# hongsukchoi/Pose2Mesh_RELEASE

Measured on NVIDIA H100. Metric: SMPL meshes/sec, higher is better.
Workload: dtype f32 (wgmma fp16x3 split, fp32 accumulate)

## Files before the change

pose2mesh_release_b200/csrc/cheb_umma.cu:

```cuda
#include <cuda.h>
#include <cuda_fp16.h>
#include <cuda_runtime.h>

#include <algorithm>
#include <cstdlib>
#include <cstring>
#include <vector>

#include "p2m_internal.h"

namespace p2m {

namespace {

constexpr int TILE_M = 128;
constexpr int FC = 32;
constexpr int A_BLOCK_BYTES = TILE_M * 128;
constexpr float W_SCALE = 64.f;
constexpr float W_INV_SCALE = 1.f / 64.f;

struct TileHeader {
  int n_rows;
  int h1;
  int nnz;
  int off_halo;
  int off_rp;
  int off_ent;
  int off_ord2;
  int bytes;
  int pad[8];
};
static_assert(sizeof(TileHeader) == 64, "header size");

inline int up16(int x) { return (x + 15) & ~15; }

__device__ __forceinline__ uint32_t smem_u32(const void* p) { return (uint32_t)__cvta_generic_to_shared(p); }

__device__ __forceinline__ void mbar_init(uint32_t bar, uint32_t count) {
  asm volatile("mbarrier.init.shared::cta.b64 [%0], %1;" ::"r"(bar), "r"(count));
}
__device__ __forceinline__ void mbar_arrive(uint32_t bar) {
  asm volatile("mbarrier.arrive.shared::cta.b64 _, [%0];" ::"r"(bar) : "memory");
}
__device__ __forceinline__ void mbar_arrive_expect_tx(uint32_t bar, uint32_t bytes) {
  asm volatile("mbarrier.arrive.expect_tx.shared::cta.b64 _, [%0], %1;" ::"r"(bar), "r"(bytes) : "memory");
}
__device__ __forceinline__ bool mbar_try_wait(uint32_t bar, uint32_t parity) {
  uint32_t ok;
  asm volatile(
      "{\n\t.reg .pred p;\n\t"
      "mbarrier.try_wait.parity.shared::cta.b64 p, [%1], %2, %3;\n\t"
      "selp.u32 %0, 1, 0, p;\n\t}"
      : "=r"(ok)
      : "r"(bar), "r"(parity), "r"(20000u)
      : "memory");
  return ok != 0;
}
__device__ __forceinline__ unsigned long long global_ns() {
  unsigned long long t;
  asm volatile("mov.u64 %0, %globaltimer;" : "=l"(t));
  return t;
}
constexpr unsigned long long MBAR_TIMEOUT_NS = 2000000000ull;
__device__ __noinline__ void mbar_timeout(volatile int* abort_flag, int* status, int code) {
  *abort_flag = 1;
  *reinterpret_cast<volatile int*>(status) = code;
  __threadfence_system();
}
__device__ __forceinline__ void mbar_wait(uint32_t bar, uint32_t parity, volatile int* abort_flag, int* status,
                                          int code) {
  if (mbar_try_wait(bar, parity)) return;
  unsigned long long t0 = 0;
  for (unsigned spin = 0;; ++spin) {
#pragma unroll 1
    for (int it = 0; it < 64; ++it) {
      if (mbar_try_wait(bar, parity)) return;
    }
    if (*abort_flag) return;
    if ((spin & 63u) == 63u) {
      const unsigned long long t = global_ns();
      if (t0 == 0) t0 = t;
      else if (t - t0 > MBAR_TIMEOUT_NS) break;
    }
  }
  mbar_timeout(abort_flag, status, code);
}
template <unsigned SLEEP_NS = 200>
__device__ __forceinline__ void mbar_wait_relaxed(uint32_t bar, uint32_t parity, volatile int* abort_flag, int* status,
                                                  int code) {
  if (mbar_try_wait(bar, parity)) return;
  unsigned long long t0 = 0;
  for (unsigned spin = 0;; ++spin) {
#pragma unroll 1
    for (int it = 0; it < 16; ++it) {
      if (mbar_try_wait(bar, parity)) return;
      __nanosleep(SLEEP_NS);
    }
    if (*abort_flag) return;
    if ((spin & 255u) == 255u) {
      const unsigned long long t = global_ns();
      if (t0 == 0) t0 = t;
      else if (t - t0 > MBAR_TIMEOUT_NS) break;
    }
  }
  mbar_timeout(abort_flag, status, code);
}
__device__ __forceinline__ void fence_barrier_init() { asm volatile("fence.mbarrier_init.release.cluster;" ::: "memory"); }
__device__ __forceinline__ void fence_async_proxy() { asm volatile("fence.proxy.async.shared::cta;" ::: "memory"); }

__device__ __forceinline__ void bulk_g2s(uint32_t dst, const void* src, uint32_t bytes, uint32_t bar) {
  asm volatile("cp.async.bulk.shared::cluster.global.mbarrier::complete_tx::bytes [%0], [%1], %2, [%3];" ::"r"(dst),
               "l"(src), "r"(bytes), "r"(bar)
               : "memory");
}
__device__ __forceinline__ void cp_async16(uint32_t dst, const void* src) {
  asm volatile("cp.async.cg.shared.global [%0], [%1], 16;" ::"r"(dst), "l"(src) : "memory");
}
__device__ __forceinline__ void cp_async16_zfill(uint32_t dst, const void* src, uint32_t src_bytes) {
  asm volatile("cp.async.cg.shared.global [%0], [%1], 16, %2;" ::"r"(dst), "l"(src), "r"(src_bytes) : "memory");
}
__device__ __forceinline__ void tma_load_2d(uint32_t dst, const CUtensorMap* tm, int c0, int c1, uint32_t bar) {
  asm volatile(
      "cp.async.bulk.tensor.2d.shared::cluster.global.mbarrier::complete_tx::bytes [%0], [%1, {%2, %3}], [%4];" ::"r"(dst),
      "l"(reinterpret_cast<uint64_t>(tm)), "r"(c0), "r"(c1), "r"(bar)
      : "memory");
}
__device__ __forceinline__ void prefetch_l2(const void* ptr) {
  asm volatile("prefetch.global.L2 [%0];" ::"l"(ptr));
}
__device__ __forceinline__ void cp_async_arrive_noinc(uint32_t bar) {
  asm volatile("cp.async.mbarrier.arrive.noinc.shared::cta.b64 [%0];" ::"r"(bar) : "memory");
}
__device__ __forceinline__ void producer_barrier() { asm volatile("bar.sync 1, 512;" ::: "memory"); }
__device__ __forceinline__ float4 lds_f4(uint32_t a) {
  float4 v;
  asm volatile("ld.shared.v4.f32 {%0, %1, %2, %3}, [%4];" : "=f"(v.x), "=f"(v.y), "=f"(v.z), "=f"(v.w) : "r"(a));
  return v;
}
__device__ __forceinline__ uint2 lds_u2(uint32_t a) {
  uint2 v;
  asm volatile("ld.shared.v2.u32 {%0, %1}, [%2];" : "=r"(v.x), "=r"(v.y) : "r"(a));
  return v;
}
__device__ __forceinline__ uint32_t lds_u16(uint32_t a) {
  unsigned short v;
  asm volatile("ld.shared.u16 %0, [%1];" : "=h"(v) : "r"(a));
  return v;
}
__device__ __forceinline__ void sts_f4(uint32_t a, const float4& v) {
  asm volatile("st.shared.v4.f32 [%0], {%1, %2, %3, %4};" ::"r"(a), "f"(v.x), "f"(v.y), "f"(v.z), "f"(v.w) : "memory");
}
__device__ __forceinline__ void sts_f2(uint32_t a, float x, float y) {
  asm volatile("st.shared.v2.f32 [%0], {%1, %2};" ::"r"(a), "f"(x), "f"(y) : "memory");
}
__device__ __forceinline__ void sts_u2(uint32_t a, const uint2& v) {
  asm volatile("st.shared.v2.u32 [%0], {%1, %2};" ::"r"(a), "r"(v.x), "r"(v.y) : "memory");
}
__device__ __forceinline__ void fma4(float4& acc, float w, const float4& x) {
  acc.x = fmaf(w, x.x, acc.x);
  acc.y = fmaf(w, x.y, acc.y);
  acc.z = fmaf(w, x.z, acc.z);
  acc.w = fmaf(w, x.w, acc.w);
}
__device__ __forceinline__ float4 cheb_t2(const float4& g, const float4& x) {
  return make_float4(fmaf(2.f, g.x, -x.x), fmaf(2.f, g.y, -x.y), fmaf(2.f, g.z, -x.z), fmaf(2.f, g.w, -x.w));
}
__device__ __forceinline__ float4 gather_row4(uint32_t ent, uint32_t e, uint32_t e1, uint32_t rows_q) {
  float4 acc0 = make_float4(0.f, 0.f, 0.f, 0.f), acc1 = acc0;
  for (; e + 3 < e1; e += 4) {
    const uint2 a0 = lds_u2(ent + e * 8), a1 = lds_u2(ent + e * 8 + 8), a2 = lds_u2(ent + e * 8 + 16),
                a3 = lds_u2(ent + e * 8 + 24);
    const float4 x0 = lds_f4(rows_q + a0.x), x1 = lds_f4(rows_q + a1.x), x2 = lds_f4(rows_q + a2.x),
                 x3 = lds_f4(rows_q + a3.x);
    fma4(acc0, __uint_as_float(a0.y), x0);
    fma4(acc1, __uint_as_float(a1.y), x1);
    fma4(acc0, __uint_as_float(a2.y), x2);
    fma4(acc1, __uint_as_float(a3.y), x3);
  }
  if (e + 1 < e1) {
    const uint2 a0 = lds_u2(ent + e * 8), a1 = lds_u2(ent + e * 8 + 8);
    const float4 x0 = lds_f4(rows_q + a0.x), x1 = lds_f4(rows_q + a1.x);
    fma4(acc0, __uint_as_float(a0.y), x0);
    fma4(acc1, __uint_as_float(a1.y), x1);
    e += 2;
  }
  if (e < e1) {
    const uint2 a0 = lds_u2(ent + e * 8);
    fma4(acc0, __uint_as_float(a0.y), lds_f4(rows_q + a0.x));
  }
  return make_float4(acc0.x + acc1.x, acc0.y + acc1.y, acc0.z + acc1.z, acc0.w + acc1.w);
}

__device__ __forceinline__ void wg_fence() { asm volatile("wgmma.fence.sync.aligned;" ::: "memory"); }
__device__ __forceinline__ void wg_commit() { asm volatile("wgmma.commit_group.sync.aligned;" ::: "memory"); }
__device__ __forceinline__ void wg_wait0() { asm volatile("wgmma.wait_group.sync.aligned 0;" ::: "memory"); }
template <int TA, int TB>
__device__ __forceinline__ void wgmma_m64n64(float (&d)[32], uint64_t desc_a, uint64_t desc_b) {
  asm volatile(
      "{\n\t.reg .pred p;\n\tsetp.ne.b32 p, 1, 0;\n\t"
      "wgmma.mma_async.sync.aligned.m64n64k16.f32.f16.f16 "
      "{%0, %1, %2, %3, %4, %5, %6, %7, %8, %9, %10, %11, %12, %13, %14, %15, "
      "%16, %17, %18, %19, %20, %21, %22, %23, %24, %25, %26, %27, %28, %29, %30, %31}, %32, %33, p, 1, 1, %34, %35;\n\t}"
      : "+f"(d[0]), "+f"(d[1]), "+f"(d[2]), "+f"(d[3]), "+f"(d[4]), "+f"(d[5]), "+f"(d[6]), "+f"(d[7]), "+f"(d[8]),
        "+f"(d[9]), "+f"(d[10]), "+f"(d[11]), "+f"(d[12]), "+f"(d[13]), "+f"(d[14]), "+f"(d[15]), "+f"(d[16]),
        "+f"(d[17]), "+f"(d[18]), "+f"(d[19]), "+f"(d[20]), "+f"(d[21]), "+f"(d[22]), "+f"(d[23]), "+f"(d[24]),
        "+f"(d[25]), "+f"(d[26]), "+f"(d[27]), "+f"(d[28]), "+f"(d[29]), "+f"(d[30]), "+f"(d[31])
      : "l"(desc_a), "l"(desc_b), "n"(TA), "n"(TB)
      : "memory");
}
template <int TA, int TB>
__device__ __forceinline__ void wgmma_m64n32(float (&d)[16], uint64_t desc_a, uint64_t desc_b) {
  asm volatile(
      "{\n\t.reg .pred p;\n\tsetp.ne.b32 p, 1, 0;\n\t"
      "wgmma.mma_async.sync.aligned.m64n32k16.f32.f16.f16 "
      "{%0, %1, %2, %3, %4, %5, %6, %7, %8, %9, %10, %11, %12, %13, %14, %15}, %16, %17, p, 1, 1, %18, %19;\n\t}"
      : "+f"(d[0]), "+f"(d[1]), "+f"(d[2]), "+f"(d[3]), "+f"(d[4]), "+f"(d[5]), "+f"(d[6]), "+f"(d[7]), "+f"(d[8]),
        "+f"(d[9]), "+f"(d[10]), "+f"(d[11]), "+f"(d[12]), "+f"(d[13]), "+f"(d[14]), "+f"(d[15])
      : "l"(desc_a), "l"(desc_b), "n"(TA), "n"(TB)
      : "memory");
// ... 28 lines not shown
struct KParams {
  const float* x;
  int in_unpool;
  int V, P, fin;
  int n_tiles;
  const unsigned char* meta;
  const int* meta_bytes;
  int meta_stride, max_h1;
  const unsigned char* wpack;
  const float* zero_row;
  EpiDev ep;
  int res_identity;
  const float* t1;
  const float* a_scale;
  long long ldy;
  int y_col0;
  float* y;
  int* status;
  long long* trace;
  int own_table;
  const float* head_wt;
  float* head_z;
  const unsigned char* apack;
  long long wslice_bytes;
  long long wblock_stride;
  int tma;
  CUtensorMap tm_x, tm_t1;
};

#ifdef P2M_UMMA_TRACE
__device__ __forceinline__ void trace_ev(const KParams& p, int role, int& n, int ev) {
  if (p.trace != nullptr && blockIdx.x == 0 && blockIdx.y == 0 && n < 512) {
    p.trace[role * 512 + n] = ((long long)ev << 48) | (clock64() & 0xFFFFFFFFFFFFll);
    ++n;
  }
}
#else
__device__ __forceinline__ void trace_ev(const KParams&, int, int&, int) {}
#endif

constexpr int W_PROD = 16;
constexpr int W_XLOAD = 16, N_XLOAD = 2, W_BLOAD = 18, W_EPI0 = 20;
constexpr int NUM_THREADS2 = 24 * 32;
constexpr int REGS_LAUNCH = 80, REGS_UTIL = 40, REGS_EPI = 120;
static_assert(128 * (REGS_EPI - REGS_LAUNCH) <= 128 * (REGS_LAUNCH - REGS_UTIL), "register pool balance");
static_assert(W_XLOAD % 4 == 0 && W_EPI0 % 4 == 0 && W_EPI0 - W_XLOAD == 4, "setmaxnreg works on aligned warpgroups");

template <int N>
__host__ __device__ constexpr int tile_rows() { return N == 128 ? 64 : TILE_M; }
template <int N, int NS, int XS, int MODE>
__global__ void __launch_bounds__(NUM_THREADS2, 1) k_cheb_conv_umma(const __grid_constant__ KParams p) {
  static_assert(N == 64 || N == 128, "one warpgroup holds the CTA's 128 x 64 or 64 x 128 accumulator in registers");
  constexpr int TM = tile_rows<N>();
  constexpr int RPT = TM / 64;
  constexpr int H = TM / 64;
  constexpr int ER = 16 * H;
  constexpr bool KT1 = (MODE == 1);
  constexpr bool plain = !KT1;
  constexpr bool XDIRECT = KT1 && NS >= 3;
  constexpr int A_BYTES = TM * 128;
  constexpr int B_BLOCK_BYTES = N * 128;
  constexpr int SLOT_BYTES = A_BYTES + B_BLOCK_BYTES;

  extern __shared__ __align__(1024) unsigned char smem_raw[];
  unsigned char* ring = smem_raw;
  float* Xs = reinterpret_cast<float*>(ring + NS * SLOT_BYTES);
  const size_t xs_stage_floats = (XDIRECT && TM == 64) ? 0 : (size_t)TM * FC;
  float* T1s = Xs + XS * xs_stage_floats;
  const size_t t1_stage_floats = (size_t)p.max_h1 * FC;
  unsigned char* meta_s =
      reinterpret_cast<unsigned char*>(T1s + (plain ? 0 : XS) * t1_stage_floats);
  uint64_t* bars = reinterpret_cast<uint64_t*>(meta_s + 2 * (size_t)p.meta_stride);
  uint64_t* b_ab_full = bars;
  uint64_t* b_ab_empty = b_ab_full + NS;
  uint64_t* b_x_full = b_ab_empty + NS;
  uint64_t* b_x_empty = b_x_full + XS;
  uint64_t* b_m_full = b_x_empty + XS;
  uint64_t* b_m_empty = b_m_full + 2;
  uint32_t* flags = reinterpret_cast<uint32_t*>(b_m_empty + 2);
  volatile int* abort_flag = reinterpret_cast<volatile int*>(flags + 1);
  float* ep_mul = reinterpret_cast<float*>(flags + 4);
  float* ep_add = ep_mul + N;
  constexpr int EC = 32;
  constexpr int STG_WARP_BYTES = N == 128 ? 4 * 16 * EC * 4 : 32 * EC * 4;
  unsigned char* epi_stage =
      reinterpret_cast<unsigned char*>((reinterpret_cast<uintptr_t>(ep_add + N) + 127) & ~(uintptr_t)127);
  int* own_s = reinterpret_cast<int*>(epi_stage + 4 * STG_WARP_BYTES);
  float* head_w_s = reinterpret_cast<float*>(own_s + 4 * 32);

  const int tid = threadIdx.x;
  const int warp = tid >> 5;
  const int lane = tid & 31;
  const int n_chunk = p.fin / FC;
  const int n_use = 3 * n_chunk;

  if (tid == 0) {
    for (int s = 0; s < NS; ++s) {
      mbar_init(smem_u32(b_ab_full + s), p.apack != nullptr ? 1 : W_PROD + 1);
      mbar_init(smem_u32(b_ab_empty + s), 4);
    }
    for (int s = 0; s < XS; ++s) {
      mbar_init(smem_u32(b_x_full + s), N_XLOAD * 32 + 1);
      mbar_init(smem_u32(b_x_empty + s), 1);
    }
    for (int s = 0; s < 2; ++s) {
      mbar_init(smem_u32(b_m_full + s), 1);
      mbar_init(smem_u32(b_m_empty + s), 1);
    }
    *abort_flag = (smem_u32(ring) & 1023u) ? 1 : 0;
    if (*abort_flag) mbar_timeout(abort_flag, p.status, 100);
    fence_barrier_init();
  }
  const float a_scale = p.a_scale ? *p.a_scale : 1.f;
  const int ecol0 = (int)blockIdx.y * N;
  for (int n = threadIdx.x; n < N; n += NUM_THREADS2) {
    const float sc = (p.ep.scale ? p.ep.scale[ecol0 + n] : 1.f) / a_scale;
    const float sh = p.ep.scale ? p.ep.shift[ecol0 + n] : 0.f;
    const float bi = p.ep.bias ? p.ep.bias[ecol0 + n] : 0.f;
    ep_mul[n] = W_INV_SCALE * sc;
    ep_add[n] = fmaf(bi, p.ep.scale ? p.ep.scale[ecol0 + n] : 1.f, sh);
  }
  if (N == 64 && p.head_z != nullptr)
    for (int i = threadIdx.x; i < 64 * 12; i += NUM_THREADS2) head_w_s[i] = p.head_wt[i];
  __syncthreads();

  if (warp >= W_XLOAD && warp < W_EPI0) {
  asm volatile("setmaxnreg.dec.sync.aligned.u32 %0;" ::"n"(REGS_UTIL));
  if (warp >= W_XLOAD && warp < W_XLOAD + N_XLOAD) {
    if (p.apack == nullptr) {
      const int lt = tid - W_XLOAD * 32;
      const int lq = lt & 7, lrg = lt >> 3;
      const int my_tiles = (p.n_tiles - (int)blockIdx.x + (int)gridDim.x - 1) / (int)gridDim.x;
      if (lt == 32 && p.tma) {
        if (!XDIRECT) asm volatile("prefetch.tensormap [%0];" ::"l"(reinterpret_cast<uint64_t>(&p.tm_x)) : "memory");
        if (KT1) asm volatile("prefetch.tensormap [%0];" ::"l"(reinterpret_cast<uint64_t>(&p.tm_t1)) : "memory");
      }
      auto fetch_meta = [&](int itf) {
        const int pat = (blockIdx.x + itf * gridDim.x) % p.P;
        const int m = itf & 1;
        mbar_wait_relaxed(smem_u32(b_m_empty + m), ((itf >> 1) & 1) ^ 1, abort_flag, p.status, 1);
        const int mbytes = p.meta_bytes[pat];
        mbar_arrive_expect_tx(smem_u32(b_m_full + m), mbytes);
        bulk_g2s(smem_u32(meta_s + (size_t)m * p.meta_stride), p.meta + (size_t)pat * p.meta_stride, mbytes,
                 smem_u32(b_m_full + m));
      };
      if (lt == 0 && my_tiles > 0) fetch_meta(0);
      const uint32_t fin_bytes = (uint32_t)p.fin * 4u;
      const int sh = p.in_unpool ? 1 : 0;
      int g2 = 0;
      int ltn = 0;
      for (int it2 = 0; it2 < my_tiles; ++it2) {
        const int tile2 = blockIdx.x + it2 * gridDim.x;
        const long long mesh_row0 = (long long)(tile2 / p.P) * p.V;
        const int m2 = it2 & 1;
        mbar_wait_relaxed(smem_u32(b_m_full + m2), (it2 >> 1) & 1, abort_flag, p.status, 8);
        const unsigned char* mb2 = meta_s + (size_t)m2 * p.meta_stride;
        const TileHeader* hdr2 = reinterpret_cast<const TileHeader*>(mb2);
        const int* halo = reinterpret_cast<const int*>(mb2 + hdr2->off_halo);
        const int h1 = hdr2->h1;
        for (int c2 = 0; c2 < n_chunk; ++c2, ++g2) {
          const int xs2 = g2 % XS;
          mbar_wait_relaxed(smem_u32(b_x_empty + xs2), ((g2 / XS) & 1) ^ 1, abort_flag, p.status, 11);
          if (lt == 0) trace_ev(p, 4, ltn, 1);
          const uint32_t xbar = smem_u32(b_x_full + xs2);
          auto stage_rows = [&](uint32_t dbase, const char* sbase, int first, int n_rows, int shift) {
            for (int i0 = first + lrg; i0 < n_rows; i0 += 32) {
              int v[4];
#pragma unroll
              for (int u = 0; u < 4; ++u) v[u] = (i0 + 8 * u < n_rows) ? halo[i0 + 8 * u] : -2;
#pragma unroll
              for (int u = 0; u < 4; ++u) {
                if (v[u] != -2) {
                  const uint32_t srow = (uint32_t)max(v[u], 0) >> shift;
                  cp_async16_zfill(dbase + (i0 + 8 * u) * 128, sbase + (uint64_t)srow * (uint64_t)fin_bytes,
                                   v[u] >= 0 ? 16u : 0u);
                }
              }
            }
          };
          const char* t1_mesh =
              reinterpret_cast<const char*>(KT1 ? p.t1 + mesh_row0 * p.fin + c2 * FC + lq * 4 : nullptr);
          const char* x_mesh = reinterpret_cast<const char*>(p.x + (mesh_row0 >> sh) * p.fin + c2 * FC + lq * 4);
          const uint32_t t1_dst = smem_u32(T1s + xs2 * t1_stage_floats) + lq * 16;
          const uint32_t x_dst = smem_u32(Xs + xs2 * xs_stage_floats) + lq * 16;
          if (p.tma) {
            if (lt == 32) {
              const int own0 = tile2 * TM;
              mbar_arrive_expect_tx(xbar, (XDIRECT ? 0 : (p.in_unpool ? TM / 2 : TM) * 128) + (KT1 ? TM * 128 : 0));
              if (!XDIRECT)
                tma_load_2d(smem_u32(Xs + xs2 * xs_stage_floats), &p.tm_x, c2 * FC, p.in_unpool ? own0 >> 1 : own0, xbar);
              if (KT1) tma_load_2d(smem_u32(T1s + xs2 * t1_stage_floats), &p.tm_t1, c2 * FC, own0, xbar);
            }
            if (KT1) stage_rows(t1_dst, t1_mesh, TM, h1, 0);
          } else {
            if (KT1) stage_rows(t1_dst, t1_mesh, 0, h1, 0);
            if (!XDIRECT) stage_rows(x_dst, x_mesh, 0, TM, sh);
            if (lt == 32) mbar_arrive(xbar);
          }
          cp_async_arrive_noinc(xbar);
          if (lt == 0) trace_ev(p, 4, ltn, 2);
          if (lt == 0 && c2 == (n_chunk > 1 ? 1 : 0) && it2 + 1 < my_tiles) fetch_meta(it2 + 1);
        }
      }
    }
  } else if (warp == W_BLOAD) {
    if (lane == 0) {
      uint32_t ucnt = 0;
      int tn = 0;
      const int uses = plain ? n_chunk : n_use;
      for (int tile = blockIdx.x; tile < p.n_tiles; tile += gridDim.x) {
        for (int u = 0; u < uses; ++u, ++ucnt) {
          const int s = ucnt % NS;
          const uint32_t par = (ucnt / NS) & 1;
          mbar_wait_relaxed(smem_u32(b_ab_empty + s), par ^ 1, abort_flag, p.status, 4);
          trace_ev(p, 1, tn, 10 + u);
          const unsigned char* wsl = p.wpack + (size_t)blockIdx.y * (size_t)p.wslice_bytes;
          if (p.apack != nullptr) {
            mbar_arrive_expect_tx(smem_u32(b_ab_full + s), B_BLOCK_BYTES + A_BYTES);
            bulk_g2s(smem_u32(ring + s * SLOT_BYTES), p.apack + ((size_t)tile * uses + u) * A_BYTES, A_BYTES,
                     smem_u32(b_ab_full + s));
          } else {
            mbar_arrive_expect_tx(smem_u32(b_ab_full + s), B_BLOCK_BYTES);
          }
          bulk_g2s(smem_u32(ring + s * SLOT_BYTES + A_BYTES), wsl + (size_t)u * (size_t)p.wblock_stride, B_BLOCK_BYTES,
                   smem_u32(b_ab_full + s));
        }
      }
    }
  }
  } else if (warp >= W_EPI0) {
    asm volatile("setmaxnreg.inc.sync.aligned.u32 %0;" ::"n"(REGS_EPI));
    const int wq = warp - W_EPI0;
    constexpr int CPR = EC / 4;
    constexpr int RPI = 32 / CPR;
    const uint32_t stg = smem_u32(epi_stage) + (uint32_t)wq * STG_WARP_BYTES;
    const int prow = lane / CPR, pc = lane % CPR;
    constexpr int NP = ER / RPI;
    int colk[2];
#pragma unroll
    for (int k = 0; k < 2; ++k) colk[k] = (int)(((uint32_t)pc ^ (uint32_t)((k * RPI + prow) & 7)) << 2);
    const int trow = (lane >> 4) * 64 + wq * 16 + (lane & 15);
    const int uses = plain ? n_chunk : n_use;
    uint32_t ucnt = 0;
    int it = 0;
    int etn = 0;
    for (int tile = blockIdx.x; tile < p.n_tiles; tile += gridDim.x, ++it) {
      const int b = tile / p.P, pat = tile - b * p.P;
      const long long mesh0 = (long long)b * p.V;
      int* own_w = own_s + wq * 32;
      {
        int v;
        if (lane >= ER) {
          v = -1;
        } else if (p.own_table) {
          v = __ldg(reinterpret_cast<const int*>(p.meta + (size_t)pat * p.meta_stride + 64) + trow);
        } else {
          v = pat * TM + trow;
          if (v >= p.V) v = -1;
        }
        __syncwarp();
        own_w[lane] = v;
        __syncwarp();
      }
      int own_v[NP];
#pragma unroll
      for (int i = 0; i < NP; ++i) own_v[i] = own_w[i * RPI + prow];
      if (p.ep.res != nullptr) {
        const int lpr = ((p.apack != nullptr ? N : p.ep.res_F) * 4 + 127) >> 7;
        for (int j = lane; j < ER * lpr; j += 32) {
          const int rr = j / lpr, ln = j - rr * lpr;
          const int vtx = own_w[rr];
          if (vtx >= 0) {
            const long long r = mesh0 + vtx;
            prefetch_l2(p.ep.res + (p.ep.res_unpool ? (r >> 1) : r) * p.ep.res_F + (p.apack != nullptr ? ecol0 : 0) + ln * 32);
          }
        }
      }
      float acc[2][32];
#pragma unroll
      for (int h = 0; h < 2; ++h)
#pragma unroll
        for (int j = 0; j < 32; ++j) acc[h][j] = 0.f;
      if (wq == 0 && lane == 0) trace_ev(p, 3, etn, 1);
      for (int u = 0; u < uses; ++u, ++ucnt) {
        const uint32_t s = ucnt % NS;
        if (wq == 0 && lane == 0) trace_ev(p, 3, etn, 4);
        mbar_wait(smem_u32(b_ab_full + s), (ucnt / NS) & 1, abort_flag, p.status, 6);
        if (wq == 0 && lane == 0) trace_ev(p, 3, etn, 5);
        const uint32_t a0 = smem_u32(ring + s * SLOT_BYTES);
        wg_fence();
#pragma unroll
        for (int h = 0; h < 2; ++h) {
          const uint64_t da = make_desc_sw128(a0 + (TM == 128 ? (uint32_t)h * (64 * 128) : 0u));
          const uint64_t db = make_desc_sw128(a0 + A_BYTES + (TM == 64 ? (uint32_t)h * (64 * 128) : 0u));
          wgmma_m64n64<0, 0>(acc[h], da + 0, db + 0);
          wgmma_m64n64<0, 0>(acc[h], da + 2, db + 2);
          wgmma_m64n64<0, 0>(acc[h], da + 4, db + 0);
          wgmma_m64n64<0, 0>(acc[h], da + 6, db + 2);
          wgmma_m64n64<0, 0>(acc[h], da + 0, db + 4);
          wgmma_m64n64<0, 0>(acc[h], da + 2, db + 6);
        }
        wg_commit();
        wg_wait0();
        __syncwarp();
        if (lane == 0) mbar_arrive(smem_u32(b_ab_empty + s));
      }
      if (wq == 0 && lane == 0) trace_ev(p, 3, etn, 2);
      auto stage_slab = [&](int cb) {
        const uint32_t sb = stg + (N == 128 ? (uint32_t)(cb / 32) * (16 * EC * 4) : 0u);
#pragma unroll
        for (int h = 0; h < H; ++h)
#pragma unroll
          for (int jj = 0; jj < 4; ++jj)
#pragma unroll
            for (int r = 0; r < 2; ++r) {
              const int lr = 16 * h + (lane >> 2) + 8 * r;
              const int cc = 8 * jj + 2 * (lane & 3);
              const int ah = TM == 128 ? h : cb / 64;
              const int j = 4 * ((TM == 128 ? cb : cb % 64) / 8 + jj) + 2 * r;
              sts_f2(sb + lr * (EC * 4) + ((((uint32_t)(cc >> 2)) ^ (uint32_t)(lr & 7)) << 4) + (cc & 3) * 4,
                     acc[ah][j], acc[ah][j + 1]);
            }
        __syncwarp();
      };
      if (N == 64 && p.head_z != nullptr) {
        float z[12];
#pragma unroll
        for (int j = 0; j < 12; ++j) z[j] = 0.f;
#pragma unroll
        for (int cb = 0; cb < N; cb += 32) {
          stage_slab(cb);
#pragma unroll
          for (int c = 0; c < 8; ++c) {
            const float4 a = lds_f4(stg + lane * (EC * 4) + (((uint32_t)c ^ (uint32_t)(lane & 7)) << 4));
            const float av[4] = {a.x, a.y, a.z, a.w};
#pragma unroll
            for (int e = 0; e < 4; ++e) {
              const int n = cb + 4 * c + e;
              float t = fmaf(av[e], ep_mul[n], ep_add[n]);
              if (p.ep.relu) t = fmaxf(t, 0.f);
              const float4 w0 = *reinterpret_cast<const float4*>(head_w_s + n * 12);
              const float4 w1 = *reinterpret_cast<const float4*>(head_w_s + n * 12 + 4);
              const float4 w2 = *reinterpret_cast<const float4*>(head_w_s + n * 12 + 8);
              z[0] = fmaf(t, w0.x, z[0]); z[1] = fmaf(t, w0.y, z[1]); z[2] = fmaf(t, w0.z, z[2]); z[3] = fmaf(t, w0.w, z[3]);
              z[4] = fmaf(t, w1.x, z[4]); z[5] = fmaf(t, w1.y, z[5]); z[6] = fmaf(t, w1.z, z[6]); z[7] = fmaf(t, w1.w, z[7]);
              z[8] = fmaf(t, w2.x, z[8]); z[9] = fmaf(t, w2.y, z[9]); z[10] = fmaf(t, w2.z, z[10]); z[11] = fmaf(t, w2.w, z[11]);
            }
          }
          __syncwarp();
        }
        if (own_w[lane] >= 0) {
          float4* zr = reinterpret_cast<float4*>(p.head_z + (mesh0 + own_w[lane]) * 12);
          zr[0] = make_float4(z[0], z[1], z[2], z[3]);
          zr[1] = make_float4(z[4], z[5], z[6], z[7]);
          zr[2] = make_float4(z[8], z[9], z[10], z[11]);
        }
      } else if (N == 128) {
#pragma unroll
        for (int cb = 0; cb < N; cb += 32) stage_slab(cb);
        const bool res_id = p.ep.res != nullptr && p.res_identity;
        float4 rv[N / 32][NP];
#pragma unroll
        for (int cb = 0; cb < N; cb += 32)
#pragma unroll
          for (int i = 0; i < NP; ++i) {
            rv[cb / 32][i] = make_float4(0.f, 0.f, 0.f, 0.f);
            if (res_id && own_v[i] >= 0) {
              const long long r = mesh0 + own_v[i];
              rv[cb / 32][i] = __ldg(reinterpret_cast<const float4*>(
                  p.ep.res + (p.ep.res_unpool ? (r >> 1) : r) * p.ep.res_F + ecol0 + cb + colk[i & 1]));
            }
          }
#pragma unroll
        for (int cb = 0; cb < N; cb += 32) {
          const uint32_t sb = stg + (uint32_t)(cb / 32) * (16 * EC * 4);
          float4 mu_k[2], ad_k[2];
#pragma unroll
          for (int k = 0; k < 2; ++k) {
            mu_k[k] = *reinterpret_cast<const float4*>(ep_mul + cb + colk[k]);
            ad_k[k] = *reinterpret_cast<const float4*>(ep_add + cb + colk[k]);
          }
#pragma unroll
          for (int i = 0; i < NP; ++i) {
            const int rr = i * RPI + prow;
            const int gn = ecol0 + cb + colk[i & 1];
            const float4 a = lds_f4(sb + rr * (EC * 4) + (pc << 4));
            const int vtx = own_v[i];
            if (vtx >= 0) {
              const float4 mu = mu_k[i & 1], ad = ad_k[i & 1];
              float o[4] = {fmaf(a.x, mu.x, ad.x), fmaf(a.y, mu.y, ad.y), fmaf(a.z, mu.z, ad.z), fmaf(a.w, mu.w, ad.w)};
              if (p.ep.relu) {
#pragma unroll
                for (int e = 0; e < 4; ++e) o[e] = fmaxf(o[e], 0.f);
              }
              const long long r = mesh0 + vtx;
              if (p.ep.res != nullptr) {
                if (p.res_identity) {
                  o[0] += rv[cb / 32][i].x; o[1] += rv[cb / 32][i].y; o[2] += rv[cb / 32][i].z; o[3] += rv[cb / 32][i].w;
                } else {
                  const float* res_row = p.ep.res + (p.ep.res_unpool ? (r >> 1) : r) * p.ep.res_F;
#pragma unroll
                  for (int e = 0; e < 4; ++e) {
                    const float l = __ldg(p.ep.lam + gn + e);
                    o[e] += (1.f - l) * __ldg(res_row + __ldg(p.ep.i0 + gn + e)) + l * __ldg(res_row + __ldg(p.ep.i1 + gn + e));
                  }
                }
              }
              *reinterpret_cast<float4*>(p.y + r * p.ldy + p.y_col0 + gn) = make_float4(o[0], o[1], o[2], o[3]);
            }
          }
        }
        __syncwarp();
      } else {
#pragma unroll
        for (int cb = 0; cb < N; cb += 32) {
          stage_slab(cb);
          float4 mu_k[2], ad_k[2];
#pragma unroll
          for (int k = 0; k < 2; ++k) {
            mu_k[k] = *reinterpret_cast<const float4*>(ep_mul + cb + colk[k]);
            ad_k[k] = *reinterpret_cast<const float4*>(ep_add + cb + colk[k]);
          }
#pragma unroll
          for (int i = 0; i < NP; ++i) {
            const int rr = i * RPI + prow;
            const int n = cb + colk[i & 1];
            const int gn = ecol0 + n;
            const float4 a = lds_f4(stg + rr * (EC * 4) + (pc << 4));
            const int vtx = own_v[i];
            if (vtx >= 0) {
              const float4 mu = mu_k[i & 1], ad = ad_k[i & 1];
              float o[4] = {fmaf(a.x, mu.x, ad.x), fmaf(a.y, mu.y, ad.y), fmaf(a.z, mu.z, ad.z), fmaf(a.w, mu.w, ad.w)};
              if (p.ep.relu) {
#pragma unroll
                for (int e = 0; e < 4; ++e) o[e] = fmaxf(o[e], 0.f);
              }
              const long long r = mesh0 + vtx;
              if (p.ep.res != nullptr) {
                const float* res_row = p.ep.res + (p.ep.res_unpool ? (r >> 1) : r) * p.ep.res_F;
                if (p.res_identity) {
                  const float4 rv = __ldg(reinterpret_cast<const float4*>(res_row + gn));
                  o[0] += rv.x; o[1] += rv.y; o[2] += rv.z; o[3] += rv.w;
                } else {
#pragma unroll
                  for (int e = 0; e < 4; ++e) {
                    const float l = __ldg(p.ep.lam + gn + e);
                    o[e] += (1.f - l) * __ldg(res_row + __ldg(p.ep.i0 + gn + e)) + l * __ldg(res_row + __ldg(p.ep.i1 + gn + e));
                  }
                }
              }
              *reinterpret_cast<float4*>(p.y + r * p.ldy + p.y_col0 + gn) = make_float4(o[0], o[1], o[2], o[3]);
            }
          }
          __syncwarp();
        }
      }
    }
  } else {
    if (p.apack == nullptr) {
    const int q = tid & 7;
    const int rg = tid >> 3;
    const uint32_t t1s_a = smem_u32(T1s);
    const uint32_t ring_a = smem_u32(ring);
    const int my_tiles = (p.n_tiles - (int)blockIdx.x + (int)gridDim.x - 1) / (int)gridDim.x;
    const int n_stage = my_tiles * n_chunk;

    uint32_t row[RPT], re[RPT], ent_a = 0;
    int ptn = 0;
    uint32_t slot = 0, spar = 0;
    uint32_t so_f[RPT], so_s[RPT];
#pragma unroll
    for (int ps = 0; ps < RPT; ++ps) row[ps] = re[ps] = so_f[ps] = so_s[ps] = 0;
    const bool odd = (rg & 1) != 0;
    auto next_slot = [&]() {
      if (++slot == (uint32_t)NS) {
        slot = 0;
        spar ^= 1u;
      }
    };

    const int xsh = (p.tma && p.in_unpool) ? 1 : 0;
    const float* xp[RPT];
#pragma unroll
    for (int ps = 0; ps < RPT; ++ps) xp[ps] = nullptr;
    int it = 0, c = -1;
    for (int g = 0; g < n_stage; ++g) {
      if (++c == n_chunk) {
        c = 0;
        ++it;
      }
      const int m = it & 1;
      const int xs = g % XS;
      float4 xd[RPT];
#pragma unroll
      for (int ps = 0; ps < RPT; ++ps) {
        xd[ps] = make_float4(0.f, 0.f, 0.f, 0.f);
        if (XDIRECT && c != 0 && xp[ps]) xd[ps] = __ldg(reinterpret_cast<const float4*>(xp[ps] + c * FC));
      }
      if (tid == 0) trace_ev(p, 0, ptn, 1);
      mbar_wait(smem_u32(b_x_full + xs), (g / XS) & 1, abort_flag, p.status, 9);
      if (tid == 0) trace_ev(p, 0, ptn, 2);

      if (c == 0) {
        mbar_wait(smem_u32(b_m_full + m), (it >> 1) & 1, abort_flag, p.status, 8);
        const unsigned char* mb = meta_s + (size_t)m * p.meta_stride;
        const TileHeader* hdr = reinterpret_cast<const TileHeader*>(mb);
        const uint32_t mb_a = smem_u32(mb);
        const uint32_t rp_a = mb_a + hdr->off_rp, ord2_a = mb_a + hdr->off_ord2;
        ent_a = mb_a + hdr->off_ent;
#pragma unroll
        for (int ps = 0; ps < RPT; ++ps) {
          row[ps] = plain ? (uint32_t)(64 * ps + rg) : lds_u16(ord2_a + 2 * (64 * ps + rg));
          re[ps] = plain ? 0u : (lds_u16(rp_a + 2 * row[ps]) | (lds_u16(rp_a + 2 * row[ps] + 2) << 16));
          const uint32_t i = row[ps];
          const uint32_t a_hi = sw128_off(i, q >> 1) + (q & 1) * 8, a_lo = sw128_off(i, 4 + (q >> 1)) + (q & 1) * 8;
          so_f[ps] = odd ? a_lo : a_hi;
          so_s[ps] = odd ? a_hi : a_lo;
        }
        if (XDIRECT) {
          const int* halo = reinterpret_cast<const int*>(mb + hdr->off_halo);
          const int sh = p.in_unpool ? 1 : 0;
          const long long mesh_row0 = (long long)((blockIdx.x + (unsigned)it * gridDim.x) / (unsigned)p.P) * p.V;
          const float* xm = p.x + (mesh_row0 >> sh) * p.fin + q * 4;
#pragma unroll
          for (int ps = 0; ps < RPT; ++ps) {
            const int v = halo[row[ps]];
            xp[ps] = (v >= 0) ? xm + (size_t)((uint32_t)v >> sh) * (uint32_t)p.fin : nullptr;
            if (xp[ps]) xd[ps] = __ldg(reinterpret_cast<const float4*>(xp[ps]));
          }
        }
      }
      const uint32_t xs_q = smem_u32(Xs + xs * xs_stage_floats) + q * 16;
      const uint32_t t1s_q = t1s_a + (uint32_t)(xs * t1_stage_floats * 4) + q * 16;
      if (plain) {
        const uint32_t s = slot;
        mbar_wait(smem_u32(b_ab_empty + s), spar ^ 1u, abort_flag, p.status, 10);
        const uint32_t ablk = ring_a + s * SLOT_BYTES;
#pragma unroll
        for (int ps = 0; ps < RPT; ++ps) {
          const uint32_t i = ps * 64 + rg;
// ... 439 lines not shown
    uint4* dst = reinterpret_cast<uint4*>(meta_s);
    const int n16 = p.meta_bytes[pat] >> 4;
    for (int i = tid; i < n16; i += 512) dst[i] = src[i];
  }
  __syncthreads();
  const TileHeader* hdr = reinterpret_cast<const TileHeader*>(meta_s);
  const int h1 = hdr->h1;
  const int* halo = reinterpret_cast<const int*>(meta_s + hdr->off_halo);
  const uint32_t mb_a = smem_u32(meta_s);
  const uint32_t rp_a = mb_a + hdr->off_rp, ent_a = mb_a + hdr->off_ent, ord2_a = mb_a + hdr->off_ord2;
  const int n_chunk = p.fin / FC;
  long long srow[4];
#pragma unroll
  for (int u = 0; u < 4; ++u) {
    const int i = rg + 64 * u;
    const int v = (i < h1) ? halo[i] : -2;
    long long r = mesh_row0 + v;
    if (p.in_unpool) r >>= 1;
    srow[u] = (v >= 0) ? r * p.fin : (long long)v;
  }
  auto stage = [&](int c) {
    if (c < n_chunk) {
      const uint32_t dst0 = smem_u32(Xs + (c % T1_STAGES) * stage_floats) + q * 16;
      const float* src0 = p.x + c * FC + q * 4;
#pragma unroll
      for (int u = 0; u < 4; ++u) {
        const int i = rg + 64 * u;
        if (srow[u] >= 0)
          cp_async16(dst0 + i * 128, src0 + srow[u]);
        else if (srow[u] == -1)
          sts_f4(dst0 + i * 128, make_float4(0.f, 0.f, 0.f, 0.f));
      }
    }
    asm volatile("cp.async.commit_group;" ::: "memory");
  };
  int vtx[2];
  uint32_t re[2];
#pragma unroll
  for (int ps = 0; ps < 2; ++ps) {
    const int i = lds_u16(ord2_a + 2 * (ps * 64 + rg));
    vtx[ps] = halo[i];
    re[ps] = lds_u16(rp_a + 2 * i) | (lds_u16(rp_a + 2 * i + 2) << 16);
  }
#pragma unroll
  for (int c = 0; c < T1_STAGES - 1; ++c) stage(c);
  for (int c = 0; c < n_chunk; ++c) {
    asm volatile("cp.async.wait_group %0;" ::"n"(T1_STAGES - 2) : "memory");
    __syncthreads();
    stage(c + T1_STAGES - 1);
    const uint32_t xs_q = smem_u32(Xs + (c % T1_STAGES) * stage_floats) + q * 16;
#pragma unroll
    for (int ps = 0; ps < 2; ++ps) {
      if (vtx[ps] >= 0) {
        const float4 acc = gather_row4(ent_a, re[ps] & 0xFFFFu, re[ps] >> 16, xs_q);
        *reinterpret_cast<float4*>(p.t1 + (mesh_row0 + vtx[ps]) * p.fin + c * FC + q * 4) = acc;
      }
    }
  }
}

__global__ void __launch_bounds__(256) k_pack_weights(const float* __restrict__ W, int fin, int fout,
                                                      unsigned char* __restrict__ out) {
  const int idx = blockIdx.x * blockDim.x + threadIdx.x;
  const int n_blocks = (fin / FC) * 3;
  const int total = n_blocks * fout * 8;
  if (idx >= total) return;
  const int j = idx & 7;
  const int n = (idx >> 3) % fout;
  const int u = (idx >> 3) / fout;
  const int c = u / 3, k = u % 3;
  const int f0 = c * FC + (j & 3) * 8;
  __align__(16) __half h[8];
#pragma unroll
  for (int e = 0; e < 8; ++e) {
    const float w = W[(size_t)n * fin * 3 + (size_t)(f0 + e) * 3 + k] * W_SCALE;
    const __half hi = __float2half_rn(w);
    h[e] = (j < 4) ? hi : __float2half_rn(w - __half2float(hi));
  }
  *reinterpret_cast<uint4*>(out + (size_t)u * fout * 128 + sw128_off(n, j)) = *reinterpret_cast<const uint4*>(h);
}

const bool g_umma_tma = [] { const char* e = std::getenv("P2M_UMMA_TMA"); return !(e && e[0] == '0'); }();

inline int epi_stage_bytes(int N) { return N == 128 ? 4 * 16 * 128 * 4 : 4 * 32 * 32 * 4; }
size_t smem_bytes_dims(int N, int NS, int XS, int max_h1, int meta_stride, bool t1_given) {
  const int tm = N == 128 ? 64 : TILE_M;
  const size_t fixed = 1024 + (size_t)NS * (tm * 128 + N * 128) + 8 * (2 * NS + 2 * XS + 8) + 16 +
                       2 * (size_t)N * 4 + 16 + 128 + (size_t)epi_stage_bytes(N) + 4 * 32 * 4 +
                       (N == 64 ? 64 * 12 * 4 : 0);
  const size_t xs_rows = (t1_given && N == 128 && NS >= 3) ? 0 : (size_t)tm;
  return fixed + (size_t)XS * (xs_rows + (t1_given ? max_h1 : 0)) * FC * 4 + 2 * (size_t)meta_stride;
}
size_t smem_bytes_for(int N, int NS, int XS, const TileBlobs& t, bool t1_given) {
  return smem_bytes_dims(N, NS, XS, t.max_h1, t.stride, t1_given);
}
constexpr size_t SMEM_LIMIT = 227 * 1024;
constexpr int CONV_N = 64;
constexpr int WIDE_N = 128;
inline int conv_n(int fout) { return fout % WIDE_N == 0 ? WIDE_N : CONV_N; }
const TileBlobs& conv_tiles(int N, const DevLevel& g, const TileSet* tiles) {
  if (tiles != nullptr) return N == WIDE_N ? tiles->m64 : *tiles;
  return N == WIDE_N ? g.meta64 : g.meta128;
}
struct ConvCfg {
  int ns, xs;
};
ConvCfg conv_cfg(int N, const TileBlobs& t, bool t1_given) {
  for (int ns = N == WIDE_N ? 6 : 3; ns >= 3; ns -= 3)
    for (int xs = 2; xs >= 1; --xs)
      if (smem_bytes_for(N, ns, xs, t, t1_given) <= SMEM_LIMIT) return {ns, xs};
  return {0, 0};
}

typedef CUresult (*TmapEncodeFn)(CUtensorMap*, CUtensorMapDataType, cuuint32_t, void*, const cuuint64_t*, const cuuint64_t*,
                                 const cuuint32_t*, const cuuint32_t*, CUtensorMapInterleave, CUtensorMapSwizzle,
                                 CUtensorMapL2promotion, CUtensorMapFloatOOBfill);
TmapEncodeFn tmap_encoder() {
  static TmapEncodeFn fn = [] {
    void* f = nullptr;
    cudaDriverEntryPointQueryResult q;
    if (cudaGetDriverEntryPoint("cuTensorMapEncodeTiled", &f, cudaEnableDefault, &q) != cudaSuccess ||
        q != cudaDriverEntryPointSuccess)
      f = nullptr;
    return reinterpret_cast<TmapEncodeFn>(f);
  }();
  return fn;
}
bool make_row_tmap(CUtensorMap* tm, const float* base, long long rows, int fin, int box_rows) {
  TmapEncodeFn enc = tmap_encoder();
  if (enc == nullptr || (reinterpret_cast<uintptr_t>(base) & 15u) != 0) return false;
  const cuuint64_t dims[2] = {(cuuint64_t)fin, (cuuint64_t)rows};
  const cuuint64_t strides[1] = {(cuuint64_t)fin * 4};
  const cuuint32_t box[2] = {(cuuint32_t)FC, (cuuint32_t)box_rows};
  const cuuint32_t estr[2] = {1, 1};
  return enc(tm, CU_TENSOR_MAP_DATA_TYPE_FLOAT32, 2, const_cast<float*>(base), dims, strides, box, estr,
             CU_TENSOR_MAP_INTERLEAVE_NONE, CU_TENSOR_MAP_SWIZZLE_NONE, CU_TENSOR_MAP_L2_PROMOTION_L2_128B,
             CU_TENSOR_MAP_FLOAT_OOB_FILL_NONE) == CUDA_SUCCESS;
}

template <int N, int NS, int XS, int MODE>
int check_launch_regs() {
  static int state = 0;
  if (state == 0) {
    cudaFuncAttributes fa;
    P2M_CUDA_OK(cudaFuncGetAttributes(&fa, k_cheb_conv_umma<N, NS, XS, MODE>));
    state = (fa.numRegs == REGS_LAUNCH) ? 1 : -1;
  }
  if (state < 0) {
    set_error("k_cheb_conv_umma was compiled with a register count other than the one its setmaxnreg split assumes");
    return P2M_ERR_CUDA;
  }
  return P2M_OK;
}

template <int N, int NS, int XS>
int launch_cfg(const UmmaConvArgs& a, int* status, const float* zero_row, int sm_count, cudaStream_t s) {
  constexpr int TM = tile_rows<N>();
  const DevLevel& g = *a.g;
  const TileBlobs& t = conv_tiles(N, g, a.tiles);
  const size_t smem = smem_bytes_for(N, NS, XS, t, !a.plain);
  auto kern = a.plain ? k_cheb_conv_umma<N, NS, XS, 0> : k_cheb_conv_umma<N, NS, XS, 1>;
  P2M_CUDA_OK(cudaFuncSetAttribute(kern, cudaFuncAttributeMaxDynamicSharedMemorySize, (int)smem));
  P2M_TRY((a.plain ? check_launch_regs<N, NS, XS, 0>() : check_launch_regs<N, NS, XS, 1>()));
  KParams p;
  p.x = a.x;
  p.in_unpool = a.in_unpool;
  p.V = g.V;
  p.P = t.n_pattern;
  p.fin = a.fin;
  p.meta = t.meta;
  p.meta_bytes = t.bytes;
  p.meta_stride = t.stride;
  p.max_h1 = t.max_h1;
  p.own_table = a.tiles != nullptr ? 1 : 0;
  p.n_tiles = a.batch * p.P;
  p.wpack = static_cast<const unsigned char*>(a.wpack);
  p.apack = nullptr;
  p.wslice_bytes = (long long)N * 128;
  p.wblock_stride = (long long)a.fout * 128;
  p.zero_row = zero_row;
  p.ep = to_dev(a.ep);
  p.res_identity = (a.ep.res != nullptr && a.ep.res_F == a.fout) ? 1 : 0;
  p.y = a.y;
  p.t1 = a.t1;
  p.a_scale = a.a_scale;
  p.ldy = a.ldy > 0 ? a.ldy : a.fout;
  p.y_col0 = a.y_col0;
  p.status = status;
  p.trace = a.trace;
  p.head_wt = a.fout == 64 ? a.head_wt : nullptr;
  p.head_z = a.fout == 64 ? a.head_z : nullptr;
  p.tma = 0;
  std::memset(&p.tm_x, 0, sizeof(p.tm_x));
  std::memset(&p.tm_t1, 0, sizeof(p.tm_t1));
  if (a.tiles == nullptr && g.V % TILE_M == 0 && g_umma_tma) {
    const long long rows = (long long)a.batch * g.V;
    bool ok = make_row_tmap(&p.tm_x, a.x, a.in_unpool ? rows / 2 : rows, a.fin, a.in_unpool ? TM / 2 : TM);
    if (ok && a.t1 != nullptr) ok = make_row_tmap(&p.tm_t1, a.t1, rows, a.fin, TM);
    p.tma = ok ? 1 : 0;
  }
  const int n_slices = a.fout / N;
  const dim3 grid(std::min(p.n_tiles, std::max(1, sm_count / n_slices)), n_slices);
  kern<<<grid, NUM_THREADS2, smem, s>>>(p);
  P2M_LAUNCH_OK();
  return P2M_OK;
}

int launch_n(const UmmaConvArgs& a, int* status, const float* zero_row, int sm_count, cudaStream_t s) {
  const int N = conv_n(a.fout);
  const ConvCfg c = conv_cfg(N, conv_tiles(N, *a.g, a.tiles), !a.plain);
  if (c.ns == 0) {
    set_error("umma_conv: tile family does not fit shared memory");
    return P2M_ERR_INVALID;
  }
  if (N == CONV_N)
    return c.xs == 2 ? launch_cfg<CONV_N, 3, 2>(a, status, zero_row, sm_count, s)
                     : launch_cfg<CONV_N, 3, 1>(a, status, zero_row, sm_count, s);
  if (c.ns == 6)
    return c.xs == 2 ? launch_cfg<WIDE_N, 6, 2>(a, status, zero_row, sm_count, s)
                     : launch_cfg<WIDE_N, 6, 1>(a, status, zero_row, sm_count, s);
  return c.xs == 2 ? launch_cfg<WIDE_N, 3, 2>(a, status, zero_row, sm_count, s)
                   : launch_cfg<WIDE_N, 3, 1>(a, status, zero_row, sm_count, s);
}

}

namespace {
void balance_store_halves(std::vector<unsigned short>* ord) {
  std::vector<unsigned short> q0, q1;
  for (unsigned short r : *ord) ((r & 4) ? q1 : q0).push_back(r);
  if (q0.size() != q1.size() || (q0.size() & 1)) return;
  size_t o = 0;
  for (size_t g = 0; g + 1 < q0.size(); g += 2) {
    (*ord)[o++] = q0[g];
    (*ord)[o++] = q0[g + 1];
    (*ord)[o++] = q1[g];
    (*ord)[o++] = q1[g + 1];
  }
}

bool make_indexed_blob(const std::vector<int>& own, int tm, const int* rowptr, const int* colidx, const float* val,
                       std::vector<int>* slot_of, std::vector<unsigned char>* blob, int* h1_out) {
  std::vector<int> halo(own);
  int n_rows = 0;
  for (int i = 0; i < tm; ++i)
    if (own[i] >= 0) {
      (*slot_of)[own[i]] = i;
      ++n_rows;
    }
  for (int i = 0; i < tm; ++i) {
    if (own[i] < 0) continue;
    for (int e = rowptr[own[i]]; e < rowptr[own[i] + 1]; ++e) {
      const int v = colidx[e];
      if ((*slot_of)[v] < 0) {
        (*slot_of)[v] = (int)halo.size();
        halo.push_back(v);
      }
    }
  }
  const int h1 = (int)halo.size();
  std::vector<unsigned short> rp(tm + 1, 0);
  std::vector<unsigned int> ent;
  for (int i = 0; i < tm; ++i) {
    if (own[i] >= 0)
      for (int e = rowptr[own[i]]; e < rowptr[own[i] + 1]; ++e) {
        unsigned int bits;
        std::memcpy(&bits, &val[e], 4);
        ent.push_back((unsigned int)(*slot_of)[colidx[e]] * 128u);
        ent.push_back(bits);
      }
    rp[i + 1] = (unsigned short)(ent.size() / 2);
  }
  for (int v : halo)
    if (v >= 0) (*slot_of)[v] = -1;
// ... 464 lines not shown
```

Before: 8683.

## Stage wide-conv epilogue rows in padded smem and move residuals/outputs with bulk copies

For the 128-column conv epilogue, each warp now loads identity-residual rows into a padded shared staging buffer with cp.async.bulk signalled by a per-warp mbarrier. It applies scale, shift, relu and the residual directly from accumulator registers into that buffer, then writes whole output rows back to global memory with bulk shared-to-global copies. This replaces per-lane float4 __ldg residual loads and scattered float4 global stores, and lets the residual fetch overlap with the epilogue's register work. In exchange it adds wait_group synchronisation, a slightly larger staging area, and a host check that rejects output or residual rows that are not 16-byte aligned.

```diff
diff --git a/pose2mesh_release_b200/csrc/cheb_umma.cu b/pose2mesh_release_b200/csrc/cheb_umma.cu
--- a/pose2mesh_release_b200/csrc/cheb_umma.cu
+++ b/pose2mesh_release_b200/csrc/cheb_umma.cu
@@ -34,6 +34,8 @@
 
 inline int up16(int x) { return (x + 15) & ~15; }
 
+constexpr int STG_ROW_BYTES = 544;
+
 __device__ __forceinline__ uint32_t smem_u32(const void* p) { return (uint32_t)__cvta_generic_to_shared(p); }
 
 __device__ __forceinline__ void mbar_init(uint32_t bar, uint32_t count) {
@@ -113,6 +115,12 @@
                "l"(src), "r"(bytes), "r"(bar)
                : "memory");
 }
+__device__ __forceinline__ void bulk_s2g(void* dst, uint32_t src, uint32_t bytes) {
+  asm volatile("cp.async.bulk.global.shared::cta.bulk_group [%0], [%1], %2;" ::"l"(dst), "r"(src), "r"(bytes) : "memory");
+}
+__device__ __forceinline__ void bulk_commit() { asm volatile("cp.async.bulk.commit_group;" ::: "memory"); }
+__device__ __forceinline__ void bulk_wait_read0() { asm volatile("cp.async.bulk.wait_group.read 0;" ::: "memory"); }
+__device__ __forceinline__ void bulk_wait0() { asm volatile("cp.async.bulk.wait_group 0;" ::: "memory"); }
 __device__ __forceinline__ void cp_async16(uint32_t dst, const void* src) {
   asm volatile("cp.async.cg.shared.global [%0], [%1], 16;" ::"r"(dst), "l"(src) : "memory");
 }
@@ -135,6 +143,11 @@
 __device__ __forceinline__ float4 lds_f4(uint32_t a) {
   float4 v;
   asm volatile("ld.shared.v4.f32 {%0, %1, %2, %3}, [%4];" : "=f"(v.x), "=f"(v.y), "=f"(v.z), "=f"(v.w) : "r"(a));
+  return v;
+}
+__device__ __forceinline__ float2 lds_f2(uint32_t a) {
+  float2 v;
+  asm volatile("ld.shared.v2.f32 {%0, %1}, [%2];" : "=f"(v.x), "=f"(v.y) : "r"(a));
   return v;
 }
 __device__ __forceinline__ uint2 lds_u2(uint32_t a) {
@@ -329,11 +342,12 @@
   float* ep_mul = reinterpret_cast<float*>(flags + 4);
   float* ep_add = ep_mul + N;
   constexpr int EC = 32;
-  constexpr int STG_WARP_BYTES = N == 128 ? 4 * 16 * EC * 4 : 32 * EC * 4;
+  constexpr int STG_WARP_BYTES = N == 128 ? 16 * STG_ROW_BYTES : 32 * EC * 4;
   unsigned char* epi_stage =
       reinterpret_cast<unsigned char*>((reinterpret_cast<uintptr_t>(ep_add + N) + 127) & ~(uintptr_t)127);
   int* own_s = reinterpret_cast<int*>(epi_stage + 4 * STG_WARP_BYTES);
   float* head_w_s = reinterpret_cast<float*>(own_s + 4 * 32);
+  uint64_t* b_res = reinterpret_cast<uint64_t*>(head_w_s);
 
   const int tid = threadIdx.x;
   const int warp = tid >> 5;
@@ -354,6 +368,8 @@
       mbar_init(smem_u32(b_m_full + s), 1);
       mbar_init(smem_u32(b_m_empty + s), 1);
     }
+    if (N == 128)
+      for (int w = 0; w < 4; ++w) mbar_init(smem_u32(b_res + w), 1);
     *abort_flag = (smem_u32(ring) & 1023u) ? 1 : 0;
     if (*abort_flag) mbar_timeout(abort_flag, p.status, 100);
     fence_barrier_init();
@@ -512,7 +528,22 @@
       int own_v[NP];
 #pragma unroll
       for (int i = 0; i < NP; ++i) own_v[i] = own_w[i * RPI + prow];
-      if (p.ep.res != nullptr) {
+      if (N == 128) {
+        if (lane < ER) bulk_wait_read0();
+        __syncwarp();
+        if (p.ep.res != nullptr && p.res_identity) {
+          const uint32_t rbar = smem_u32(b_res + wq);
+          const int n_valid = __popc(__ballot_sync(0xFFFFFFFFu, lane < ER && own_w[lane] >= 0));
+          if (lane == 0) mbar_arrive_expect_tx(rbar, (uint32_t)n_valid * (N * 4));
+          __syncwarp();
+          if (lane < ER && own_w[lane] >= 0) {
+            const long long r = mesh0 + own_w[lane];
+            bulk_g2s(stg + lane * STG_ROW_BYTES, p.ep.res + (p.ep.res_unpool ? (r >> 1) : r) * p.ep.res_F + ecol0, N * 4,
+                     rbar);
+          }
+        }
+      }
+      if (p.ep.res != nullptr && (N == 64 || !p.res_identity)) {
         const int lpr = ((p.apack != nullptr ? N : p.ep.res_F) * 4 + 127) >> 7;
         for (int j = lane; j < ER * lpr; j += 32) {
           const int rr = j / lpr, ln = j - rr * lpr;
@@ -554,7 +585,6 @@
       }
       if (wq == 0 && lane == 0) trace_ev(p, 3, etn, 2);
       auto stage_slab = [&](int cb) {
-        const uint32_t sb = stg + (N == 128 ? (uint32_t)(cb / 32) * (16 * EC * 4) : 0u);
 #pragma unroll
         for (int h = 0; h < H; ++h)
 #pragma unroll
@@ -563,10 +593,9 @@
             for (int r = 0; r < 2; ++r) {
               const int lr = 16 * h + (lane >> 2) + 8 * r;
               const int cc = 8 * jj + 2 * (lane & 3);
-              const int ah = TM == 128 ? h : cb / 64;
-              const int j = 4 * ((TM == 128 ? cb : cb % 64) / 8 + jj) + 2 * r;
-              sts_f2(sb + lr * (EC * 4) + ((((uint32_t)(cc >> 2)) ^ (uint32_t)(lr & 7)) << 4) + (cc & 3) * 4,
-                     acc[ah][j], acc[ah][j + 1]);
+              const int j = 4 * (cb / 8 + jj) + 2 * r;
+              sts_f2(stg + lr * (EC * 4) + ((((uint32_t)(cc >> 2)) ^ (uint32_t)(lr & 7)) << 4) + (cc & 3) * 4,
+                     acc[h][j], acc[h][j + 1]);
             }
         __syncwarp();
       };
@@ -603,61 +632,62 @@
           zr[2] = make_float4(z[8], z[9], z[10], z[11]);
         }
       } else if (N == 128) {
-#pragma unroll
-        for (int cb = 0; cb < N; cb += 32) stage_slab(cb);
         const bool res_id = p.ep.res != nullptr && p.res_identity;
-        float4 rv[N / 32][NP];
-#pragma unroll
-        for (int cb = 0; cb < N; cb += 32)
-#pragma unroll
-          for (int i = 0; i < NP; ++i) {
-            rv[cb / 32][i] = make_float4(0.f, 0.f, 0.f, 0.f);
-            if (res_id && own_v[i] >= 0) {
-              const long long r = mesh0 + own_v[i];
-              rv[cb / 32][i] = __ldg(reinterpret_cast<const float4*>(
-                  p.ep.res + (p.ep.res_unpool ? (r >> 1) : r) * p.ep.res_F + ecol0 + cb + colk[i & 1]));
+        if (res_id) mbar_wait(smem_u32(b_res + wq), (uint32_t)it & 1u, abort_flag, p.status, 12);
+        if (wq == 0 && lane == 0) trace_ev(p, 3, etn, 21);
+#pragma unroll
+        for (int h = 0; h < 2; ++h)
+#pragma unroll
+          for (int jg = 0; jg < 8; ++jg) {
+            const int n = 64 * h + 8 * jg + 2 * (lane & 3);
+            const float2 mu = *reinterpret_cast<const float2*>(ep_mul + n);
+            const float2 ad = *reinterpret_cast<const float2*>(ep_add + n);
+#pragma unroll
+            for (int r = 0; r < 2; ++r) {
+              const int j = 4 * jg + 2 * r;
+              const uint32_t a = stg + ((lane >> 2) + 8 * r) * STG_ROW_BYTES + n * 4;
+              float o0 = fmaf(acc[h][j], mu.x, ad.x), o1 = fmaf(acc[h][j + 1], mu.y, ad.y);
+              if (p.ep.relu) {
+                o0 = fmaxf(o0, 0.f);
+                o1 = fmaxf(o1, 0.f);
+              }
+              if (res_id) {
+                const float2 rv = lds_f2(a);
+                o0 += rv.x;
+                o1 += rv.y;
+              }
+              sts_f2(a, o0, o1);
             }
           }
-#pragma unroll
-        for (int cb = 0; cb < N; cb += 32) {
-          const uint32_t sb = stg + (uint32_t)(cb / 32) * (16 * EC * 4);
-          float4 mu_k[2], ad_k[2];
-#pragma unroll
-          for (int k = 0; k < 2; ++k) {
-            mu_k[k] = *reinterpret_cast<const float4*>(ep_mul + cb + colk[k]);
-            ad_k[k] = *reinterpret_cast<const float4*>(ep_add + cb + colk[k]);
-          }
-#pragma unroll
-          for (int i = 0; i < NP; ++i) {
-            const int rr = i * RPI + prow;
-            const int gn = ecol0 + cb + colk[i & 1];
-            const float4 a = lds_f4(sb + rr * (EC * 4) + (pc << 4));
-            const int vtx = own_v[i];
+        if (p.ep.res != nullptr && !p.res_identity) {
+          __syncwarp();
+          const int gn = ecol0 + 4 * lane;
+          for (int rr = 0; rr < ER; ++rr) {
+            const int vtx = own_w[rr];
             if (vtx >= 0) {
-              const float4 mu = mu_k[i & 1], ad = ad_k[i & 1];
-              float o[4] = {fmaf(a.x, mu.x, ad.x), fmaf(a.y, mu.y, ad.y), fmaf(a.z, mu.z, ad.z), fmaf(a.w, mu.w, ad.w)};
-              if (p.ep.relu) {
-#pragma unroll
-                for (int e = 0; e < 4; ++e) o[e] = fmaxf(o[e], 0.f);
+              const long long r = mesh0 + vtx;
+              const float* res_row = p.ep.res + (p.ep.res_unpool ? (r >> 1) : r) * p.ep.res_F;
+              const uint32_t a = stg + rr * STG_ROW_BYTES + lane * 16;
+              const float4 v = lds_f4(a);
+              float o[4] = {v.x, v.y, v.z, v.w};
+#pragma unroll
+              for (int e = 0; e < 4; ++e) {
+                const float l = __ldg(p.ep.lam + gn + e);
+                o[e] += (1.f - l) * __ldg(res_row + __ldg(p.ep.i0 + gn + e)) + l * __ldg(res_row + __ldg(p.ep.i1 + gn + e));
               }
-              const long long r = mesh0 + vtx;
-              if (p.ep.res != nullptr) {
-                if (p.res_identity) {
-                  o[0] += rv[cb / 32][i].x; o[1] += rv[cb / 32][i].y; o[2] += rv[cb / 32][i].z; o[3] += rv[cb / 32][i].w;
-                } else {
-                  const float* res_row = p.ep.res + (p.ep.res_unpool ? (r >> 1) : r) * p.ep.res_F;
-#pragma unroll
-                  for (int e = 0; e < 4; ++e) {
-                    const float l = __ldg(p.ep.lam + gn + e);
-                    o[e] += (1.f - l) * __ldg(res_row + __ldg(p.ep.i0 + gn + e)) + l * __ldg(res_row + __ldg(p.ep.i1 + gn + e));
-                  }
-                }
-              }
-              *reinterpret_cast<float4*>(p.y + r * p.ldy + p.y_col0 + gn) = make_float4(o[0], o[1], o[2], o[3]);
+              sts_f4(a, make_float4(o[0], o[1], o[2], o[3]));
             }
           }
         }
+        if (wq == 0 && lane == 0) trace_ev(p, 3, etn, 22);
+        fence_async_proxy();
         __syncwarp();
+        if (lane < ER) {
+          if (own_w[lane] >= 0)
+            bulk_s2g(p.y + (mesh0 + own_w[lane]) * p.ldy + p.y_col0 + ecol0, stg + lane * STG_ROW_BYTES, N * 4);
+          bulk_commit();
+        }
+        if (wq == 0 && lane == 0) trace_ev(p, 3, etn, 23);
       } else {
 #pragma unroll
         for (int cb = 0; cb < N; cb += 32) {
@@ -703,6 +733,7 @@
         }
       }
     }
+    if (N == 128 && lane < ER) bulk_wait0();
   } else {
     if (p.apack == nullptr) {
     const int q = tid & 7;
@@ -1308,12 +1339,12 @@
 
 const bool g_umma_tma = [] { const char* e = std::getenv("P2M_UMMA_TMA"); return !(e && e[0] == '0'); }();
 
-inline int epi_stage_bytes(int N) { return N == 128 ? 4 * 16 * 128 * 4 : 4 * 32 * 32 * 4; }
+inline int epi_stage_bytes(int N) { return N == 128 ? 4 * 16 * STG_ROW_BYTES : 4 * 32 * 32 * 4; }
 size_t smem_bytes_dims(int N, int NS, int XS, int max_h1, int meta_stride, bool t1_given) {
   const int tm = N == 128 ? 64 : TILE_M;
   const size_t fixed = 1024 + (size_t)NS * (tm * 128 + N * 128) + 8 * (2 * NS + 2 * XS + 8) + 16 +
                        2 * (size_t)N * 4 + 16 + 128 + (size_t)epi_stage_bytes(N) + 4 * 32 * 4 +
-                       (N == 64 ? 64 * 12 * 4 : 0);
+                       (N == 64 ? 64 * 12 * 4 : 4 * 8);
   const size_t xs_rows = (t1_given && N == 128 && NS >= 3) ? 0 : (size_t)tm;
   return fixed + (size_t)XS * (xs_rows + (t1_given ? max_h1 : 0)) * FC * 4 + 2 * (size_t)meta_stride;
 }
@@ -1416,6 +1447,14 @@
   p.trace = a.trace;
   p.head_wt = a.fout == 64 ? a.head_wt : nullptr;
   p.head_z = a.fout == 64 ? a.head_z : nullptr;
+  if (N == WIDE_N) {
+    const bool y_ok = (reinterpret_cast<uintptr_t>(p.y) & 15u) == 0 && (p.ldy * 4) % 16 == 0 && (p.y_col0 * 4) % 16 == 0;
+    const bool res_ok = !p.res_identity || ((reinterpret_cast<uintptr_t>(p.ep.res) & 15u) == 0 && (p.ep.res_F * 4) % 16 == 0);
+    if (!y_ok || !res_ok) {
+      set_error("umma_conv: the 128-column epilogue needs 16-byte aligned output and identity-residual rows");
+      return P2M_ERR_INVALID;
+    }
+  }
   p.tma = 0;
   std::memset(&p.tm_x, 0, sizeof(p.tm_x));
   std::memset(&p.tm_t1, 0, sizeof(p.tm_t1));
```

Result: faster. 9042 (median of 6 runs) (+4.1%).
